# NVIDIA-Genomics-Research/GenomeWorks

Measured on AMD Instinct MI355X. Metric: cudapoa consensus GCUPS, 1024-window short-read batch (static band 256, 32 reads <= 1024 bp), higher is better.
Workload: dtype int16; 1 GPU; BASELINE configs[2]: cudapoa single-batch consensus, 1024 windows x 32 reads, backbone 960 bp, <=48 sub/24 ins/24 del, BatchConfig(1024,32,256,static_band), scores 8/-6/-8; windows_per_gpu=1024, cells_per_gpu=10990578176, parallelism=index-split x1

## Files before the change

### genomeworks_amd/csrc/poa_forward_moves.h

```cpp
#pragma once

namespace gwhip
{

constexpr int kKindShift = 60;
constexpr uint32_t kMoveHoriz = 1;

__device__ __forceinline__ uint32_t pk_mad_u16_vsv(uint32_t a, uint32_t s, uint32_t c)
{
    uint32_t d;
    asm("v_pk_mad_u16 %0, %1, %2, %3" : "=v"(d) : "v"(a), "s"(s), "v"(c));
    return d;
}
__device__ __forceinline__ uint32_t pk_mad_u16_vvs(uint32_t a, uint32_t b, uint32_t s)
{
    uint32_t d;
    asm("v_pk_mad_u16 %0, %1, %2, %3" : "=v"(d) : "v"(a), "v"(b), "s"(s));
    return d;
}
__device__ __forceinline__ void gstore_nt_u64(void* p, uint32_t lo, uint32_t hi)
{
    u32x2 v;
    v.x = lo; v.y = hi;
    __builtin_nontemporal_store(v, reinterpret_cast<u32x2*>(p));
}
__device__ __forceinline__ void gstore_u16_lane0_below(const void* vptr, uint32_t v)
{
    asm volatile("s_mov_b64 exec, 1\n\tglobal_store_short %0, %1, off offset:-2\n\ts_mov_b64 exec, -1" ::"v"(vptr), "v"(v) : "memory");
}

template <int MAXD = kPkMaxDist, bool TBRULES = false>
__device__ __forceinline__ int32_t classify_kinds(RowInfo<true>* rowinfo, int32_t graph_count, int lane, const uint64_t* xpred, int32_t dbg = 0)
{
    int32_t first_moved = graph_count + 1;
    for (int32_t r = 1 + lane; r <= graph_count; r += kWave)
    {
        RowInfo<true> ri  = rowinfo[r];
        const int32_t cnt = ri.cnt(), bs = ri.bs();
        uint64_t kind     = 4;
        const uint64_t xe  = (cnt > 3 && cnt <= 6 && xpred != nullptr) ? xpred[r & 255] : 0ull;
        const bool many_ok = cnt > 3 && cnt <= 6 && xpred_hit(xe, r, cnt) && !(dbg & (1 << 30));
        if (cnt >= 1 && (cnt <= 3 || many_ok))
        {
            bool ok    = true;
            int32_t d0 = 0, pbs0 = 0;
            for (int32_t k = 0; k < cnt; k++)
            {
                const int32_t p   = k < 3 ? ri.pred(k) : xpred_row(xe, k);
                const int32_t d   = r - p;
                const RowInfo<true> pri = rowinfo[p];
                const int32_t pbs = pri.bs();
                ok                = ok && d >= 1 && d <= MAXD && (bs - pbs) <= kPkGuardCols && (bs == 0 || pbs > 0);
                if constexpr (TBRULES) ok = ok && !(pri.cnt() == 0 && pbs > 0);
                if (k == 0) { d0 = d; pbs0 = pbs; }
            }
            if (ok) kind = cnt > 1 ? 3 : ((d0 == 1 && pbs0 == bs) ? 0 : ((d0 == 1 && bs - pbs0 == kCellsPerLane) ? 1 : 2));
        }
        if ((dbg & 1024) && kind <= 1) kind = 2;
        if ((dbg & 32768) && kind == 1) kind = 2;
        if ((dbg & 512) && (kind == 2 || kind == 3)) kind = 4;
        if ((dbg & 2048) && kind <= 1) kind = 4;
        ri.w       = (ri.w & ~(7ull << kKindShift)) | (kind << kKindShift);
        rowinfo[r] = ri;
        if (bs > 0) first_moved = min(first_moved, r);
    }
    for (int off = 32; off > 0; off >>= 1) first_moved = min(first_moved, __shfl_xor(first_moved, off));
    return __builtin_amdgcn_readfirstlane(first_moved);
}

constexpr uint64_t kRowScoresInHbm = 1ull << 63;
template <typename IdT>
__device__ __forceinline__ void mark_score_rows(const GraphView<IdT>& g, RowInfo<true>* rowinfo, int32_t graph_count, int lane, bool all_rows)
{
    auto mark = [&](int32_t row) {
        __hip_atomic_fetch_or(reinterpret_cast<uint32_t*>(&rowinfo[row].w) + 1, 0x80000000u, __ATOMIC_RELAXED, __HIP_MEMORY_SCOPE_WORKGROUP);
    };
    for (int32_t r = 1 + lane; r <= graph_count; r += kWave)
    {
        const uint64_t w    = rowinfo[r].w;
        const uint32_t kind = (uint32_t)(w >> kKindShift) & 7u;
        const int32_t cnt   = (int32_t)((w >> 8) & 0x3fu);
        const bool reads_or_recomputes = kind >= 4u || cnt > 3;
        if (reads_or_recomputes || ((w >> 14) & 1u) != 0 || all_rows) mark(r);
        if (reads_or_recomputes)
        {
            const int32_t node_id = cnt > 3 ? (int32_t)g.sorted_poa[r - 1] : 0;
            for (int32_t k = 0; k < cnt; k++)
                mark(k < 3 ? (int32_t)((w >> (24 + 12 * k)) & 0xfffu) : (int32_t)g.node_id_to_pos[g.incoming_edges[(int64_t)node_id * kEdges + k]] + 1);
        }
    }
    wave_sync();
}
__device__ __forceinline__ bool row_recompute_safe(uint64_t w)
{
    return ((uint32_t)(w >> kKindShift) & 7u) >= 4u || ((w >> 8) & 0x3fu) > 3u || ((w >> 15) & 0x1ffu) == 0u;
}

template <typename IdT, int BW>
__device__ __forceinline__ void banded_forward_moves(const GraphView<IdT>& g, RowInfo<true>* rowinfo, int32_t graph_count,
                                                     const uint8_t* lds_read, int16_t* scores, uint8_t* moves, uint8_t* ring,
                                                     const uint64_t* xpred, int32_t max_column, int32_t gap_score,
                                                     int32_t mismatch_score, int32_t match_score, int32_t dbg,
                                                     uint64_t* prof_acc, bool store_all = true)
{
    const bool abl       = (dbg & (1 << 14)) != 0;
    const bool st_scores = !(abl && (dbg & (1 << 26))), st_moves = !(abl && (dbg & (1 << 27)));
    const bool ab_ring = !(abl && (dbg & (1 << 20))), ab_guard = !(abl && (dbg & (1 << 19))), ab_scan = !(abl && (dbg & (1 << 18))),
               ab_moves = !(abl && (dbg & (1 << 17))), ab_rows = !(abl && (dbg & (1 << 16)));
    const int32_t ksel = prof_acc ? ((dbg >> 28) & 7) - 1 : -1;
    const bool kcount  = (dbg & (1 << 12)) != 0;
    uint64_t kacc      = 0;
    static_assert(BW == 128 || BW == 256, "band widths of the packed pass");
    constexpr int32_t band_width = BW;
    constexpr int32_t stride     = band_width + kRightPad;
    constexpr int kBandLanes     = BW / kCellsPerLane;
    const int lane               = threadIdx.x & (kWave - 1);
    const bool band_lane         = lane < kBandLanes;
    const int32_t lane4 = lane * 4, lane8 = lane * 8;
    const int32_t min_score = Limits<int16_t>::min / 2;

    const int32_t first_moved = classify_kinds(rowinfo, graph_count, lane, xpred, dbg);
    wave_sync();
    mark_score_rows<IdT>(g, rowinfo, graph_count, lane, store_all);

    const uint32_t MIN2   = pin_vgpr(pk_dup(min_score));
    const uint32_t SENT2  = pin_vgpr(pk_dup(kPkSentinel));
    const uint32_t GAP2   = pin_vgpr(pk_dup(gap_score));
    const uint32_t MAT2   = pin_vgpr(pk_dup(match_score));
    const uint32_t DIF2   = pin_vgpr(pk_dup(mismatch_score - match_score));
    const uint32_t ONE2   = pin_vgpr(0x00010001u);
    const uint32_t THREE2 = pin_vgpr(0x00030003u);
    const uint32_t NEG1   = pin_vgpr(0xffffffffu);
    const uint32_t K01 = pk_make((lane4 + 0) * gap_score, (lane4 + 1) * gap_score);
    const uint32_t K23 = pk_make((lane4 + 2) * gap_score, (lane4 + 3) * gap_score);
    const uint32_t ring_base = lds_addr(ring);
    const uint32_t read_base = lds_addr(lds_read);
    const uint32_t guard_off  = lane < 16 ? (uint32_t)(2 * BW) : (lane == 16 ? (uint32_t)-136 : (uint32_t)(120 - 16 * lane));
    const bool is_lane16      = lane == 16;
    const bool is_lane63      = lane == kBandLanes - 1;
    const uint32_t move_keep  = lane == 0 ? 0xffffff00u : 0xffffffffu;
    const uint32_t GUARD_HI_MIN = pin_vgpr(is_lane16 ? (((uint32_t)kPkSentinel & 0xffffu) | ((uint32_t)min_score << 16)) : pk_dup(kPkSentinel));
    const uint32_t S0X_MIN      = (uint32_t)min_score << 16;

    uint32_t P01 = pk_make((lane4 + 1) * gap_score, (lane4 + 2) * gap_score);
    uint32_t P23 = pk_make((lane4 + 3) * gap_score, (lane4 + 4) * gap_score);
    int32_t prev_rel0 = 0;
    uint32_t rd4  = lds_load_u32(read_base + lane4);
    uint32_t rd4n = lds_load_u32(read_base + lane4 + 4);
    uint32_t a1   = (uint32_t)lane8;
    uint32_t ga   = (a1 + guard_off) & (kPkSlotBytes - 1);
    uint8_t* const score_base = reinterpret_cast<uint8_t*>(scores) + lane8 + 2 * (1 + kRelShift);
    uint8_t* move_ptr  = moves + lane4 + (1 + kRelShift);

    if (BW == 256 || band_lane) lds_store_u64(ring_base + a1, P01, P23);
    lds_store_guard(ring_base + ga, SENT2, is_lane16 ? (((uint32_t)kPkSentinel & 0xffffu) | (0u << 16)) : SENT2);

    auto scan_row = [&](uint32_t s01, uint32_t s23, int32_t cu) {
        const uint32_t u01 = pk_sub(s01, K01), u23 = pk_sub(s23, K23);
        const uint32_t pm01 = pk_max(u01, (u01 << 16) | 0x8000u);
        const uint32_t pm23 = pk_max(u23, (u23 << 16) | 0x8000u);
        const int32_t m3    = (int32_t)pk_max(pm01, pm23) >> 16;
        const int32_t incl  = ab_scan ? wave_inclusive_max(m3) : m3;
        const int32_t excl  = max(wave_shr1(incl, cu), cu);
        const uint32_t ex2  = __builtin_amdgcn_perm((uint32_t)excl, (uint32_t)excl, 0x01000100u);
        const uint32_t m1b  = __builtin_amdgcn_perm(pm01, pm01, 0x03020302u);
        P01 = pk_add(pk_max(pm01, ex2), K01);
        P23 = pk_add(pk_max(pk_max(pm23, m1b), ex2), K23);
    };
    auto nz = [&](uint32_t a, uint32_t b) -> uint32_t { return pk_min_u16(pk_sub(a, b), ONE2); };
    auto costs = [&](uint32_t base4, uint32_t& c01, uint32_t& c23) {
        const uint32_t x   = rd4 ^ base4;
        const uint32_t x01 = __builtin_amdgcn_perm(0u, x, 0x0c010c00u);
        const uint32_t x23 = __builtin_amdgcn_perm(0u, x, 0x0c030c02u);
        c01 = pk_mad_u16(pk_min_u16(x01, ONE2), DIF2, MAT2);
        c23 = pk_mad_u16(pk_min_u16(x23, ONE2), DIF2, MAT2);
    };
    auto from_pred = [&](uint32_t s0x, uint32_t q01, uint32_t q23, uint32_t c01, uint32_t c23, uint32_t& D01, uint32_t& D23,
                         uint32_t& V01, uint32_t& V23) {
        D01 = pk_add(__builtin_amdgcn_alignbit(q01, s0x, 16), c01);
        D23 = pk_add(__builtin_amdgcn_alignbit(q23, q01, 16), c23);
        V01 = pk_add(q01, GAP2);
        V23 = pk_add(q23, GAP2);
    };
    auto store_row = [&](auto bs0_tag, int32_t r, int32_t rel0_val, uint32_t mv4, bool scores_to_hbm) {
        constexpr bool BS0 = decltype(bs0_tag)::value;
        move_ptr += stride;
        const uint32_t sbase = ring_base + (((uint32_t)r & (kPkSlots - 1)) * kPkSlotBytes);
        if (BS0 || __builtin_expect(scores_to_hbm, 0))
        {
            uint8_t* score_ptr = score_base + (uint32_t)r * (uint32_t)(stride * 2);
            if (st_scores && (BW == 256 || band_lane)) gstore_nt_u64(score_ptr, P01, P23);
            if constexpr (BS0) gstore_u16_lane0_below(score_ptr, (uint32_t)rel0_val);
        }
        if (ab_ring && (BW == 256 || band_lane)) lds_store_u64(sbase + a1, P01, P23);
        if constexpr (BS0)
        {
            const uint32_t rel0pk = ((uint32_t)kPkSentinel & 0xffffu) | ((uint32_t)rel0_val << 16);
            if (ab_guard) lds_store_guard(sbase + ga, SENT2, is_lane16 ? rel0pk : SENT2);
            prev_rel0 = rel0_val;
        }
        else if (ab_guard)
            lds_store_guard(sbase + ga, SENT2, GUARD_HI_MIN);
        if (st_moves && (BW == 256 || band_lane)) *reinterpret_cast<uint32_t*>(move_ptr) = mv4;
    };
    auto pack_moves = [&](uint32_t m01, uint32_t m23) -> uint32_t {
        return __builtin_amdgcn_perm(m23, m01, 0x06040200u) & move_keep;
    };

    auto general_row = [&](int32_t r, int32_t& prev_rel0_io) {
        const RowInfo<true> ri = uniform_row(rowinfo[r]);
        const int32_t bs       = ri.bs();
        const uint32_t base    = (uint32_t)ri.base();
        const int32_t prev_bs  = r > 1 ? uniform_row(rowinfo[r - 1]).bs() : 0;
        a1   = (uint32_t)(2 * bs + lane8) & (kPkSlotBytes - 1);
        ga   = (a1 + guard_off) & (kPkSlotBytes - 1);
        rd4  = lds_load_u32(read_base + bs + lane4);
        rd4n = lds_load_u32(read_base + bs + lane4 + 4);
        const int32_t pred_count = ri.cnt();
        const int32_t c          = bs + lane4;
        const int32_t cp0 = ((rd4 & 0xff) == base) ? match_score : mismatch_score;
        const int32_t cp1 = (((rd4 >> 8) & 0xff) == base) ? match_score : mismatch_score;
        const int32_t cp2 = (((rd4 >> 16) & 0xff) == base) ? match_score : mismatch_score;
        const int32_t cp3 = ((rd4 >> 24) == base) ? match_score : mismatch_score;
        const int32_t R0 = pk_lo(P01), R1 = pk_hi(P01), R2 = pk_lo(P23), R3 = pk_hi(P23);
        bool synced = false;
        auto from_regs = [&](int32_t& t0, int32_t& t1, int32_t& t2, int32_t& t3) {
            const int32_t q    = (bs - prev_bs) >> 2;
            const int32_t pend = min(prev_bs + band_width - kCellsPerLane, max_column);
            const int src      = lane + q;
            const int32_t from_left = __shfl(R3, src - 1);
            const int32_t S0        = (q == 0 && lane == 0) ? prev_rel0_io : from_left;
            const int32_t S1 = __shfl(R0, src), S2 = __shfl(R1, src), S3 = __shfl(R2, src), S4 = __shfl(R3, src);
            const bool valid = c <= pend;
            t0 = valid ? max(S0 + cp0, S1 + gap_score) : min_score;
            t1 = valid ? max(S1 + cp1, S2 + gap_score) : min_score;
            t2 = valid ? max(S2 + cp2, S3 + gap_score) : min_score;
            t3 = valid ? max(S3 + cp3, S4 + gap_score) : min_score;
        };
        auto from_hbm = [&](int32_t prow, int32_t& t0, int32_t& t1, int32_t& t2, int32_t& t3) {
            const int32_t pbs  = prow == 0 ? 0 : uniform_row(rowinfo[prow]).bs();
            const int32_t pend = min(pbs + band_width - kCellsPerLane, max_column);
            const bool valid   = !(c > pend || c < pbs);
            if (!synced) { wave_sync(); synced = true; }
            const int16_t* rowp = scores + (int64_t)prow * stride + (valid ? (c - pbs) : 0) + kRelShift;
            int32_t S0 = rowp[0];
            const Quad<int16_t> qd = *reinterpret_cast<const Quad<int16_t>*>(rowp + 1);
            const int32_t S1 = qd.v[0], S2 = qd.v[1], S3 = qd.v[2], S4 = qd.v[3];
            if (pbs > 0 && c == pbs) S0 = min_score;
            t0 = valid ? max(S0 + cp0, S1 + gap_score) : min_score;
            t1 = valid ? max(S1 + cp1, S2 + gap_score) : min_score;
            t2 = valid ? max(S2 + cp2, S3 + gap_score) : min_score;
            t3 = valid ? max(S3 + cp3, S4 + gap_score) : min_score;
        };
        auto rel0_of = [&](int32_t prow) -> int32_t {
            if (prow == r - 1) return prev_rel0_io;
            const int32_t pbs = prow == 0 ? 0 : uniform_row(rowinfo[prow]).bs();
            if (pbs > 0) return min_score;
            if (!synced) { wave_sync(); synced = true; }
            return wave_first((int32_t)scores[(int64_t)prow * stride + kRelShift]);
        };
        const int32_t node_id = (pred_count > 3) ? (int32_t)g.sorted_poa[r - 1] : 0;
        auto pred_row = [&](int32_t p) -> int32_t {
            if (pred_count == 0) return 0;
            if (p < 3) return ri.pred(p);
            return wave_first((int32_t)g.node_id_to_pos[g.incoming_edges[(int64_t)node_id * kEdges + p]] + 1);
        };
        int32_t fe = 0, rel0_val = min_score;
        if (pred_count == 0)
        {
            if (bs == 0) rel0_val = gap_score;
        }
        else
        {
            if (bs > kCellsPerLane && pred_count == 1)
                fe = min_score + gap_score;
            else
            {
                int32_t penalty = min_score;
                for (int32_t p = 0; p < pred_count; p++) penalty = max(penalty, rel0_of(pred_row(p)));
                fe = penalty + gap_score;
            }
            if (bs == 0) rel0_val = fe;
        }
        int32_t s0 = 0, s1 = 0, s2 = 0, s3 = 0;
        const int32_t np = max(pred_count, 1);
        for (int32_t p = 0; p < np; p++)
        {
            const int32_t prow = pred_row(p);
            int32_t t0, t1, t2, t3;
            if (prow == r - 1) from_regs(t0, t1, t2, t3);
            else from_hbm(prow, t0, t1, t2, t3);
            if (p == 0) { s0 = t0; s1 = t1; s2 = t2; s3 = t3; }
            else { s0 = max(s0, t0); s1 = max(s1, t1); s2 = max(s2, t2); s3 = max(s3, t3); }
        }
        scan_row(pk_make(s0, s1), pk_make(s2, s3), fe + gap_score);
        uint8_t* score_ptr = score_base + (uint32_t)r * (uint32_t)(stride * 2);
        move_ptr += stride;
        const uint32_t sbase  = ring_base + (((uint32_t)r & (kPkSlots - 1)) * kPkSlotBytes);
        const uint32_t rel0pk = ((uint32_t)kPkSentinel & 0xffffu) | ((uint32_t)rel0_val << 16);
        if (BW == 256 || band_lane)
        {
            *reinterpret_cast<uint2*>(score_ptr) = make_uint2(P01, P23);
            lds_store_u64(sbase + a1, P01, P23);
        }
        lds_store_guard(sbase + ga, SENT2, is_lane16 ? rel0pk : SENT2);
        if (bs == 0) gstore_u16_lane0_below(score_ptr, (uint32_t)rel0_val);
        if (BW == 256 || band_lane) *reinterpret_cast<uint32_t*>(move_ptr) = 0u;
        prev_rel0_io = rel0_val;
    };

    auto reg_row = [&](auto bs0_tag, auto moved_tag, int32_t r, uint32_t d0, uint32_t base4, bool scores_to_hbm) {
        constexpr bool BS0   = decltype(bs0_tag)::value;
        constexpr bool MOVED = decltype(moved_tag)::value;
        uint32_t s0x, q01, q23;
        if constexpr (!MOVED)
        {
            s0x = (uint32_t)wave_shr1((int32_t)P23, BS0 ? (int32_t)((uint32_t)prev_rel0 << 16) : (int32_t)S0X_MIN);
            q01 = P01; q23 = P23;
        }
        else
        {
            s0x  = P23;
            q01  = (uint32_t)wave_shl1((int32_t)P01, (int32_t)pk_dup(kPkSentinel));
            q23  = (uint32_t)wave_shl1((int32_t)P23, (int32_t)pk_dup(kPkSentinel));
            a1   = (a1 + 8) & (kPkSlotBytes - 1);
            ga   = (ga + 8) & (kPkSlotBytes - 1);
            rd4  = rd4n;
            rd4n = lds_load_u32(read_base + (((d0 >> 3) & 0x1ffu) << 2) + lane4 + 4);
        }
        int32_t cu = min_score + 2 * gap_score, rel0_val = min_score;
        if constexpr (BS0)
        {
            rel0_val = max(min_score, prev_rel0) + gap_score;
            cu       = rel0_val + gap_score;
        }
        uint32_t c01, c23, D01, D23, V01, V23;
        costs(base4, c01, c23);
        from_pred(s0x, q01, q23, c01, c23, D01, D23, V01, V23);
        uint32_t s01 = pk_max(D01, V01), s23 = pk_max(D23, V23);
        if constexpr (MOVED)
        {
            s01 = is_lane63 ? MIN2 : s01;
            s23 = is_lane63 ? MIN2 : s23;
        }
        scan_row(s01, s23, cu);
        const uint32_t m01 = pk_mad_u16(nz(P01, D01), pk_mad_u16(nz(P01, V01), NEG1, NEG1), THREE2);
        const uint32_t m23 = pk_mad_u16(nz(P23, D23), pk_mad_u16(nz(P23, V23), NEG1, NEG1), THREE2);
        uint32_t mv4 = ab_moves ? pack_moves(m01, m23) : 0u;
        if constexpr (MOVED) mv4 = is_lane63 ? 0u : mv4;
        store_row(bs0_tag, r, rel0_val, mv4, scores_to_hbm);
    };

    auto run_rows = [&](auto bs0_tag, int32_t r_from, int32_t r_to) {
        constexpr bool BS0 = decltype(bs0_tag)::value;
        int32_t r = r_from;
        while (r <= r_to)
        {
            const int32_t r0   = r;
            uint32_t D0v, D1v;
            {
                const int32_t rr    = min(r0 + lane, graph_count);
                const uint64_t w    = rowinfo[rr].w;
                const uint32_t kind = (uint32_t)(w >> kKindShift) & 7u;
                const uint32_t cnt  = (uint32_t)(w >> 8) & 0x3fu;
                const uint32_t bs4  = (uint32_t)(w >> 15) & 0x1ffu;
                const uint32_t p0 = (uint32_t)(w >> 24) & 0xfffu, p1 = (uint32_t)(w >> 36) & 0xfffu, p2 = (uint32_t)(w >> 48) & 0xfffu;
                const uint32_t slots = (p0 & 7u) | ((p1 & 7u) << 3) | ((p2 & 7u) << 6);
                const uint32_t dists = (((uint32_t)rr - p0) & 7u) | ((((uint32_t)rr - p1) & 7u) << 3) | ((((uint32_t)rr - p2) & 7u) << 6);
                D0v = kind | (bs4 << 3) | (slots << 12) | (dists << 21) | ((cnt <= 3 ? cnt : 0u) << 30);
                D1v = ((uint32_t)w & 0xffu) * 0x01010101u;
            }
            D0v = (r0 + lane <= r_to) ? D0v : 7u;
            const uint64_t need64 = BS0 ? ~0ull : __ballot((rowinfo[min(r0 + lane, graph_count)].w & kRowScoresInHbm) != 0);
            int32_t k      = 0;
            uint32_t d0    = (uint32_t)__builtin_amdgcn_readlane((int32_t)D0v, 0);
            uint32_t base4 = (uint32_t)__builtin_amdgcn_readlane((int32_t)D1v, 0);
            uint32_t kind  = d0 & 7u;
            auto advance = [&]() {
                r++;
                k++;
                const uint32_t nd = (uint32_t)__builtin_amdgcn_readlane((int32_t)D0v, k & (kWave - 1));
                base4 = (uint32_t)__builtin_amdgcn_readlane((int32_t)D1v, k & (kWave - 1));
                d0    = k == kWave ? 7u : nd;
                kind  = d0 & 7u;
            };
            for (;;)
            {
                const uint64_t t_k0 = ksel == 0 ? clock64() : 0;
                const int32_t r_k0  = r;
                while (kind == 0)
                {
                    reg_row(bs0_tag, std::false_type{}, r, d0, base4, ((need64 >> k) & 1ull) != 0);
                    advance();
                }
                if (ksel == 0) kacc += kcount ? (uint64_t)(r - r_k0) : clock64() - t_k0;
                if (kind == 7u) break;
                const int32_t kind_now = (int32_t)min(kind, 4u);
                const uint64_t t_kx    = ksel == kind_now ? clock64() : 0;
                const bool scores_to_hbm = ((need64 >> k) & 1ull) != 0;
                if (kind == 1)
                    reg_row(bs0_tag, std::true_type{}, r, d0, base4, scores_to_hbm);
                else if (kind <= 3)
                {
                    const uint32_t bs = ((d0 >> 3) & 0x1ffu) << 2;
                    a1 = (2u * bs + (uint32_t)lane8) & (kPkSlotBytes - 1);
                    ga = (a1 + guard_off) & (kPkSlotBytes - 1);
                    const uint32_t a0 = (a1 - 4) & (kPkSlotBytes - 1);
                    const uint32_t b0 = ring_base + (((d0 >> 12) & 7u) * kPkSlotBytes);
                    const uint32_t sent16 = (uint32_t)kPkSentinel & 0xffffu;
                    const uint32_t dd0 = (d0 >> 21) & 7u;
                    if (kind == 2)
                    {
                        const uint32_t x0 = lds_load_u32(b0 + a0);
                        const uint2 q0    = lds_load_u64(b0 + a1);
                        rd4  = lds_load_u32(read_base + bs + lane4);
                        rd4n = lds_load_u32(read_base + bs + lane4 + 4);
                        int32_t cu = min_score + 2 * gap_score, rel0_val = min_score;
                        if constexpr (BS0)
                        {
                            rel0_val = max(min_score, (int32_t)(int16_t)wave_first((int32_t)(lds_load_u32(b0 + kPkSlotBytes - 4) >> 16))) + gap_score;
                            cu       = rel0_val + gap_score;
                        }
                        uint32_t c01, c23, D01, D23, V01, V23;
                        costs(base4, c01, c23);
                        from_pred(x0, q0.x, q0.y, c01, c23, D01, D23, V01, V23);
                        const bool outside = (q0.x & 0xffffu) == sent16;
                        const uint32_t s01 = pk_max(D01, V01), s23 = pk_max(D23, V23);
                        scan_row(outside ? MIN2 : s01, outside ? MIN2 : s23, cu);
                        const uint32_t cD = pk_dup((int32_t)(2u * dd0 + 1u)), cV = pk_dup(1 - (int32_t)(2u * dd0));
                        const uint32_t m01 = pk_mad_u16_vvs(nz(P01, D01), pk_mad_u16_vsv(nz(P01, V01), cV, NEG1), cD);
                        const uint32_t m23 = pk_mad_u16_vvs(nz(P23, D23), pk_mad_u16_vsv(nz(P23, V23), cV, NEG1), cD);
                        const uint32_t mv4 = outside ? 0u : pack_moves(m01, m23);
                        store_row(bs0_tag, r, rel0_val, mv4, scores_to_hbm);
                    }
                    else
                    {
                        const uint32_t cnt3    = d0 >> 30;
                        const int32_t cnt      = cnt3 == 2 ? 2 : 3;
                        const uint32_t b1 = ring_base + (((d0 >> 15) & 7u) * kPkSlotBytes);
                        const uint32_t b2 = cnt > 2 ? ring_base + (((d0 >> 18) & 7u) * kPkSlotBytes) : b0;
                        const uint32_t dd1 = (d0 >> 24) & 7u, dd2 = (d0 >> 27) & 7u;
                        const uint32_t x0 = lds_load_u32(b0 + a0);
                        const uint2 q0    = lds_load_u64(b0 + a1);
                        const uint32_t x1 = lds_load_u32(b1 + a0);
                        const uint2 q1    = lds_load_u64(b1 + a1);
                        uint32_t x2 = 0;
                        uint2 q2 = make_uint2(0, 0);
                        if (cnt > 2)
                        {
                            x2 = lds_load_u32(b2 + a0);
                            q2 = lds_load_u64(b2 + a1);
                        }
                        rd4  = lds_load_u32(read_base + bs + lane4);
                        rd4n = lds_load_u32(read_base + bs + lane4 + 4);
                        int32_t fe = min_score + gap_score;
                        if constexpr (BS0)
                        {
                            int32_t pen = max(min_score, (int32_t)(int16_t)wave_first((int32_t)(lds_load_u32(b0 + kPkSlotBytes - 4) >> 16)));
                            pen = max(pen, (int32_t)(int16_t)wave_first((int32_t)(lds_load_u32(b1 + kPkSlotBytes - 4) >> 16)));
                            if (cnt > 2) pen = max(pen, (int32_t)(int16_t)wave_first((int32_t)(lds_load_u32(b2 + kPkSlotBytes - 4) >> 16)));
                            fe = pen + gap_score;
                        }
                        uint32_t c01, c23;
                        costs(base4, c01, c23);
                        uint32_t D0a, D0b, V0a, V0b, D1a, D1b, V1a, V1b;
                        from_pred(x0, q0.x, q0.y, c01, c23, D0a, D0b, V0a, V0b);
                        from_pred(x1, q1.x, q1.y, c01, c23, D1a, D1b, V1a, V1b);
                        const bool out0 = (q0.x & 0xffffu) == sent16, out1 = (q1.x & 0xffffu) == sent16;
                        bool undecided  = out0 | out1;
                        D0a = out0 ? MIN2 : D0a; D0b = out0 ? MIN2 : D0b; V0a = out0 ? MIN2 : V0a; V0b = out0 ? MIN2 : V0b;
                        D1a = out1 ? MIN2 : D1a; D1b = out1 ? MIN2 : D1b; V1a = out1 ? MIN2 : V1a; V1b = out1 ? MIN2 : V1b;
                        uint32_t bD01 = pk_max(D0a, D1a), bD23 = pk_max(D0b, D1b), bV01 = pk_max(V0a, V1a), bV23 = pk_max(V0b, V1b);
                        const uint32_t mD0 = pk_dup((int32_t)(2u * dd0 + 1u)), mV0 = pk_dup((int32_t)(2u * dd0));
                        const uint32_t E1  = pk_dup(2 * ((int32_t)dd1 - (int32_t)dd0));
                        uint32_t A01, A23, B01, B23;
                        if (cnt > 2)
                        {
                            uint32_t D2a, D2b, V2a, V2b;
                            from_pred(x2, q2.x, q2.y, c01, c23, D2a, D2b, V2a, V2b);
                            const bool out2 = (q2.x & 0xffffu) == sent16;
                            undecided       = undecided | out2;
                            D2a = out2 ? MIN2 : D2a; D2b = out2 ? MIN2 : D2b; V2a = out2 ? MIN2 : V2a; V2b = out2 ? MIN2 : V2b;
                            bD01 = pk_max(bD01, D2a); bD23 = pk_max(bD23, D2b); bV01 = pk_max(bV01, V2a); bV23 = pk_max(bV23, V2b);
                            const uint32_t E2  = pin_vgpr(pk_dup(2 * ((int32_t)dd2 - (int32_t)dd1)));
                            const uint32_t E1v = pin_vgpr(E1);
                            A01 = pk_mad_u16_vvs(nz(bD01, D0a), pk_mad_u16(nz(bD01, D1a), E2, E1v), mD0);
                            A23 = pk_mad_u16_vvs(nz(bD23, D0b), pk_mad_u16(nz(bD23, D1b), E2, E1v), mD0);
                            B01 = pk_mad_u16_vvs(nz(bV01, V0a), pk_mad_u16(nz(bV01, V1a), E2, E1v), mV0);
                            B23 = pk_mad_u16_vvs(nz(bV23, V0b), pk_mad_u16(nz(bV23, V1b), E2, E1v), mV0);
                        }
                        else
                        {
                            const uint32_t E1v = pin_vgpr(E1);
                            A01 = pk_mad_u16_vvs(nz(bD01, D0a), E1v, mD0); A23 = pk_mad_u16_vvs(nz(bD23, D0b), E1v, mD0);
                            B01 = pk_mad_u16_vvs(nz(bV01, V0a), E1v, mV0); B23 = pk_mad_u16_vvs(nz(bV23, V0b), E1v, mV0);
                        }
                        if (cnt3 == 0)
                        {
                            const uint64_t xe     = wave_first64(xpred[r & 255]);
                            const int32_t cnt_all = (int32_t)((xe >> 13) & 63u);
                            uint32_t xD01 = MIN2, xD23 = MIN2, xV01 = MIN2, xV23 = MIN2;
                            int32_t pen_x = min_score;
                            for (int32_t kk = 3; kk < cnt_all; kk++)
                            {
                                const uint32_t bk = ring_base + (((uint32_t)xpred_row(xe, kk) & 7u) * kPkSlotBytes);
                                const uint32_t xk = lds_load_u32(bk + a0);
                                const uint2 qk    = lds_load_u64(bk + a1);
                                uint32_t Da, Db, Va, Vb;
                                from_pred(xk, qk.x, qk.y, c01, c23, Da, Db, Va, Vb);
                                const bool outk = (qk.x & 0xffffu) == sent16;
                                undecided       = undecided | outk;
                                xD01 = pk_max(xD01, outk ? MIN2 : Da); xD23 = pk_max(xD23, outk ? MIN2 : Db);
                                xV01 = pk_max(xV01, outk ? MIN2 : Va); xV23 = pk_max(xV23, outk ? MIN2 : Vb);
                                if constexpr (BS0) pen_x = max(pen_x, (int32_t)(int16_t)wave_first((int32_t)(lds_load_u32(bk + kPkSlotBytes - 4) >> 16)));
                            }
                            if constexpr (BS0) fe = max(fe - gap_score, pen_x) + gap_score;
                            const uint32_t fD01 = pk_max(bD01, xD01), fD23 = pk_max(bD23, xD23), fV01 = pk_max(bV01, xV01), fV23 = pk_max(bV23, xV23);
                            A01 = pk_mad_u16(nz(bD01, fD01), pk_sub(0u, A01), A01); A23 = pk_mad_u16(nz(bD23, fD23), pk_sub(0u, A23), A23);
                            B01 = pk_mad_u16(nz(bV01, fV01), pk_sub(0u, B01), B01); B23 = pk_mad_u16(nz(bV23, fV23), pk_sub(0u, B23), B23);
                            bD01 = fD01; bD23 = fD23; bV01 = fV01; bV23 = fV23;
                        }
                        const int32_t rel0_val = BS0 ? fe : min_score;
                        scan_row(pk_max(bD01, bV01), pk_max(bD23, bV23), fe + gap_score);
                        auto move_of = [&](uint32_t H, uint32_t bD, uint32_t bV, uint32_t A, uint32_t B) -> uint32_t {
                            const uint32_t t1 = pk_mad_u16(nz(H, bV), pk_sub(ONE2, B), B);
                            return pk_mad_u16(nz(H, bD), pk_sub(t1, A), A);
                        };
                        const uint32_t m01 = move_of(P01, bD01, bV01, A01, B01);
                        const uint32_t m23 = move_of(P23, bD23, bV23, A23, B23);
                        const uint32_t mv4 = undecided ? 0u : pack_moves(m01, m23);
                        store_row(bs0_tag, r, rel0_val, mv4, scores_to_hbm);
                    }
                }
                else
                {
                    general_row(r, prev_rel0);
                    if constexpr (!BS0) prev_rel0 = min_score;
                }
                if (ksel == kind_now) kacc += kcount ? 1 : clock64() - t_kx;
                advance();
            }
        }
    };

    const int32_t bs0_end = min(first_moved - 1, graph_count);
    if (!ab_rows) return;
    run_rows(std::true_type{}, 1, bs0_end);
    run_rows(std::false_type{}, bs0_end + 1, graph_count);
    if (ksel >= 0 && lane == 0) *prof_acc += kacc;
}

}
```

Baseline: 395.3 GCUPS.

## Replace per-row LDS guard stores with precomputed band-shift lane predicates

For rows not starting at band column zero, the kernel no longer writes sentinel guard words into the LDS ring on every row. Out-of-band and left-neighbour conditions are instead derived from the band-start shift between each row and its predecessors, precomputed per row into a packed register and broadcast with readlane. This drops one LDS store and the guard-address bookkeeping per row, at the cost of extra rowinfo loads and lane-compare logic in the predecessor path, with a correctness risk if the shift-based predicates differ from the sentinel semantics.

```diff
diff --git a/genomeworks_amd/csrc/poa_forward_moves.h b/genomeworks_amd/csrc/poa_forward_moves.h
--- a/genomeworks_amd/csrc/poa_forward_moves.h
+++ b/genomeworks_amd/csrc/poa_forward_moves.h
@@ -139,8 +139,7 @@
     const bool is_lane16      = lane == 16;
     const bool is_lane63      = lane == kBandLanes - 1;
     const uint32_t move_keep  = lane == 0 ? 0xffffff00u : 0xffffffffu;
-    const uint32_t GUARD_HI_MIN = pin_vgpr(is_lane16 ? (((uint32_t)kPkSentinel & 0xffffu) | ((uint32_t)min_score << 16)) : pk_dup(kPkSentinel));
-    const uint32_t S0X_MIN      = (uint32_t)min_score << 16;
+    const uint32_t S0X_MIN    = (uint32_t)min_score << 16;
 
     uint32_t P01 = pk_make((lane4 + 1) * gap_score, (lane4 + 2) * gap_score);
     uint32_t P23 = pk_make((lane4 + 3) * gap_score, (lane4 + 4) * gap_score);
@@ -148,12 +147,12 @@
     uint32_t rd4  = lds_load_u32(read_base + lane4);
     uint32_t rd4n = lds_load_u32(read_base + lane4 + 4);
     uint32_t a1   = (uint32_t)lane8;
-    uint32_t ga   = (a1 + guard_off) & (kPkSlotBytes - 1);
+    const uint32_t ga0 = ((uint32_t)lane8 + guard_off) & (kPkSlotBytes - 1);
     uint8_t* const score_base = reinterpret_cast<uint8_t*>(scores) + lane8 + 2 * (1 + kRelShift);
     uint8_t* move_ptr  = moves + lane4 + (1 + kRelShift);
 
     if (BW == 256 || band_lane) lds_store_u64(ring_base + a1, P01, P23);
-    lds_store_guard(ring_base + ga, SENT2, is_lane16 ? (((uint32_t)kPkSentinel & 0xffffu) | (0u << 16)) : SENT2);
+    lds_store_guard(ring_base + ga0, SENT2, is_lane16 ? (((uint32_t)kPkSentinel & 0xffffu) | (0u << 16)) : SENT2);
 
     auto scan_row = [&](uint32_t s01, uint32_t s23, int32_t cu) {
         const uint32_t u01 = pk_sub(s01, K01), u23 = pk_sub(s23, K23);
@@ -196,11 +195,9 @@
         if constexpr (BS0)
         {
             const uint32_t rel0pk = ((uint32_t)kPkSentinel & 0xffffu) | ((uint32_t)rel0_val << 16);
-            if (ab_guard) lds_store_guard(sbase + ga, SENT2, is_lane16 ? rel0pk : SENT2);
+            if (ab_guard) lds_store_guard(sbase + ga0, SENT2, is_lane16 ? rel0pk : SENT2);
             prev_rel0 = rel0_val;
         }
-        else if (ab_guard)
-            lds_store_guard(sbase + ga, SENT2, GUARD_HI_MIN);
         if (st_moves && (BW == 256 || band_lane)) *reinterpret_cast<uint32_t*>(move_ptr) = mv4;
     };
     auto pack_moves = [&](uint32_t m01, uint32_t m23) -> uint32_t {
@@ -213,7 +210,6 @@
         const uint32_t base    = (uint32_t)ri.base();
         const int32_t prev_bs  = r > 1 ? uniform_row(rowinfo[r - 1]).bs() : 0;
         a1   = (uint32_t)(2 * bs + lane8) & (kPkSlotBytes - 1);
-        ga   = (a1 + guard_off) & (kPkSlotBytes - 1);
         rd4  = lds_load_u32(read_base + bs + lane4);
         rd4n = lds_load_u32(read_base + bs + lane4 + 4);
         const int32_t pred_count = ri.cnt();
@@ -303,7 +299,7 @@
             *reinterpret_cast<uint2*>(score_ptr) = make_uint2(P01, P23);
             lds_store_u64(sbase + a1, P01, P23);
         }
-        lds_store_guard(sbase + ga, SENT2, is_lane16 ? rel0pk : SENT2);
+        lds_store_guard(sbase + ((a1 + guard_off) & (kPkSlotBytes - 1)), SENT2, is_lane16 ? rel0pk : SENT2);
         if (bs == 0) gstore_u16_lane0_below(score_ptr, (uint32_t)rel0_val);
         if (BW == 256 || band_lane) *reinterpret_cast<uint32_t*>(move_ptr) = 0u;
         prev_rel0_io = rel0_val;
@@ -324,7 +320,6 @@
             q01  = (uint32_t)wave_shl1((int32_t)P01, (int32_t)pk_dup(kPkSentinel));
             q23  = (uint32_t)wave_shl1((int32_t)P23, (int32_t)pk_dup(kPkSentinel));
             a1   = (a1 + 8) & (kPkSlotBytes - 1);
-            ga   = (ga + 8) & (kPkSlotBytes - 1);
             rd4  = rd4n;
             rd4n = lds_load_u32(read_base + (((d0 >> 3) & 0x1ffu) << 2) + lane4 + 4);
         }
@@ -357,7 +352,7 @@
         while (r <= r_to)
         {
             const int32_t r0   = r;
-            uint32_t D0v, D1v;
+            uint32_t D0v, D1v, D2v = 0;
             {
                 const int32_t rr    = min(r0 + lane, graph_count);
                 const uint64_t w    = rowinfo[rr].w;
@@ -369,6 +364,16 @@
                 const uint32_t dists = (((uint32_t)rr - p0) & 7u) | ((((uint32_t)rr - p1) & 7u) << 3) | ((((uint32_t)rr - p2) & 7u) << 6);
                 D0v = kind | (bs4 << 3) | (slots << 12) | (dists << 21) | ((cnt <= 3 ? cnt : 0u) << 30);
                 D1v = ((uint32_t)w & 0xffu) * 0x01010101u;
+                if constexpr (!BS0)
+                {
+                    const uint32_t np = min(cnt, 3u);
+                    auto field = [&](uint32_t k, uint32_t pk) -> uint32_t {
+                        const uint32_t pbs4 = (uint32_t)(rowinfo[k < np ? min((int32_t)pk, graph_count) : rr].w >> 15) & 0x1ffu;
+                        const uint32_t dq   = (bs4 - pbs4) & 15u;
+                        return (((uint32_t)kBandLanes - dq) << (8 * k)) | ((dq == 0u ? 1u : 0u) << (24 + k));
+                    };
+                    D2v = field(0, p0) | field(1, p1) | field(2, p2);
+                }
             }
             D0v = (r0 + lane <= r_to) ? D0v : 7u;
             const uint64_t need64 = BS0 ? ~0ull : __ballot((rowinfo[min(r0 + lane, graph_count)].w & kRowScoresInHbm) != 0);
@@ -404,11 +409,18 @@
                 {
                     const uint32_t bs = ((d0 >> 3) & 0x1ffu) << 2;
                     a1 = (2u * bs + (uint32_t)lane8) & (kPkSlotBytes - 1);
-                    ga = (a1 + guard_off) & (kPkSlotBytes - 1);
                     const uint32_t a0 = (a1 - 4) & (kPkSlotBytes - 1);
                     const uint32_t b0 = ring_base + (((d0 >> 12) & 7u) * kPkSlotBytes);
-                    const uint32_t sent16 = (uint32_t)kPkSentinel & 0xffffu;
                     const uint32_t dd0 = (d0 >> 21) & 7u;
+                    const uint32_t d2 = BS0 ? 0u : (uint32_t)__builtin_amdgcn_readlane((int32_t)D2v, k & (kWave - 1));
+                    auto beyond = [&](uint32_t qx, uint32_t first_lane_beyond) -> bool {
+                        if constexpr (BS0) return (qx & 0xffffu) == ((uint32_t)kPkSentinel & 0xffffu);
+                        else return (uint32_t)lane >= first_lane_beyond;
+                    };
+                    auto left_of = [&](uint32_t x, uint32_t same_start) -> uint32_t {
+                        if constexpr (BS0) return x;
+                        else return (uint32_t)lane < same_start ? S0X_MIN : x;
+                    };
                     if (kind == 2)
                     {
                         const uint32_t x0 = lds_load_u32(b0 + a0);
@@ -423,8 +435,8 @@
                         }
                         uint32_t c01, c23, D01, D23, V01, V23;
                         costs(base4, c01, c23);
-                        from_pred(x0, q0.x, q0.y, c01, c23, D01, D23, V01, V23);
-                        const bool outside = (q0.x & 0xffffu) == sent16;
+                        from_pred(left_of(x0, (d2 >> 24) & 1u), q0.x, q0.y, c01, c23, D01, D23, V01, V23);
+                        const bool outside = beyond(q0.x, d2 & 0xffu);
                         const uint32_t s01 = pk_max(D01, V01), s23 = pk_max(D23, V23);
                         scan_row(outside ? MIN2 : s01, outside ? MIN2 : s23, cu);
                         const uint32_t cD = pk_dup((int32_t)(2u * dd0 + 1u)), cV = pk_dup(1 - (int32_t)(2u * dd0));
@@ -464,9 +476,9 @@
                         uint32_t c01, c23;
                         costs(base4, c01, c23);
                         uint32_t D0a, D0b, V0a, V0b, D1a, D1b, V1a, V1b;
-                        from_pred(x0, q0.x, q0.y, c01, c23, D0a, D0b, V0a, V0b);
-                        from_pred(x1, q1.x, q1.y, c01, c23, D1a, D1b, V1a, V1b);
-                        const bool out0 = (q0.x & 0xffffu) == sent16, out1 = (q1.x & 0xffffu) == sent16;
+                        from_pred(left_of(x0, (d2 >> 24) & 1u), q0.x, q0.y, c01, c23, D0a, D0b, V0a, V0b);
+                        from_pred(left_of(x1, (d2 >> 25) & 1u), q1.x, q1.y, c01, c23, D1a, D1b, V1a, V1b);
+                        const bool out0 = beyond(q0.x, d2 & 0xffu), out1 = beyond(q1.x, (d2 >> 8) & 0xffu);
                         bool undecided  = out0 | out1;
                         D0a = out0 ? MIN2 : D0a; D0b = out0 ? MIN2 : D0b; V0a = out0 ? MIN2 : V0a; V0b = out0 ? MIN2 : V0b;
                         D1a = out1 ? MIN2 : D1a; D1b = out1 ? MIN2 : D1b; V1a = out1 ? MIN2 : V1a; V1b = out1 ? MIN2 : V1b;
@@ -477,8 +489,8 @@
                         if (cnt > 2)
                         {
                             uint32_t D2a, D2b, V2a, V2b;
-                            from_pred(x2, q2.x, q2.y, c01, c23, D2a, D2b, V2a, V2b);
-                            const bool out2 = (q2.x & 0xffffu) == sent16;
+                            from_pred(left_of(x2, (d2 >> 26) & 1u), q2.x, q2.y, c01, c23, D2a, D2b, V2a, V2b);
+                            const bool out2 = beyond(q2.x, (d2 >> 16) & 0xffu);
                             undecided       = undecided | out2;
                             D2a = out2 ? MIN2 : D2a; D2b = out2 ? MIN2 : D2b; V2a = out2 ? MIN2 : V2a; V2b = out2 ? MIN2 : V2b;
                             bD01 = pk_max(bD01, D2a); bD23 = pk_max(bD23, D2b); bV01 = pk_max(bV01, V2a); bV23 = pk_max(bV23, V2b);
@@ -503,12 +515,14 @@
                             int32_t pen_x = min_score;
                             for (int32_t kk = 3; kk < cnt_all; kk++)
                             {
-                                const uint32_t bk = ring_base + (((uint32_t)xpred_row(xe, kk) & 7u) * kPkSlotBytes);
+                                const int32_t prow = xpred_row(xe, kk);
+                                const uint32_t bk = ring_base + (((uint32_t)prow & 7u) * kPkSlotBytes);
                                 const uint32_t xk = lds_load_u32(bk + a0);
                                 const uint2 qk    = lds_load_u64(bk + a1);
+                                const uint32_t dq = BS0 ? 0u : (bs - (uint32_t)uniform_row(rowinfo[prow]).bs()) >> 2;
                                 uint32_t Da, Db, Va, Vb;
-                                from_pred(xk, qk.x, qk.y, c01, c23, Da, Db, Va, Vb);
-                                const bool outk = (qk.x & 0xffffu) == sent16;
+                                from_pred(left_of(xk, dq == 0u ? 1u : 0u), qk.x, qk.y, c01, c23, Da, Db, Va, Vb);
+                                const bool outk = beyond(qk.x, (uint32_t)kBandLanes - dq);
                                 undecided       = undecided | outk;
                                 xD01 = pk_max(xD01, outk ? MIN2 : Da); xD23 = pk_max(xD23, outk ? MIN2 : Db);
                                 xV01 = pk_max(xV01, outk ? MIN2 : Va); xV23 = pk_max(xV23, outk ? MIN2 : Vb);
```

Result: no change. 397.7 GCUPS, median of 6 (+0.6%).
